# cteufel13/VisualOdometry

Measured on AMD Instinct MI355X. Metric: BA GN-iters/sec at 50 poses×20k landmarks; descriptor-match Mpairs/sec, higher is better.
Workload: dtype f64; 1 GPU; cfg3: synthetic sliding-window BA window, 50 poses x 20000 landmarks, 83108 observations (seed 3, KITTI K, first 2 poses fixed, lambda=1.0); one step = one full GN iteration; poses=50, landmarks=20000, observations=83108, parallelism=landmark-sharded x1, k1_variant=0

## Files before the change

visualodometry_amd/_lib.py:

```python

from __future__ import annotations

import ctypes as C
import os
import threading
from pathlib import Path

LIB_PATH = Path(os.environ.get("VO_LIB_PATH") or Path(__file__).resolve().parent / "lib" / "libvo_hip.so")
HEADER = Path(__file__).resolve().parents[1] / "include" / "vo_hip.h"
TEST_HEADER = HEADER.with_name("vo_hip_testing.h")

VO_OK = 0
VO_ERR_ARG = -1
VO_ERR_HIP = -2
VO_ERR_NOT_SPD = -3
VO_ERR_RCCL = -4
VO_ERR_NOMEM = -5
VO_ERR_STATE = -6
VO_ERR_NODEV = -7
VO_MATCH_DEVICE_PTRS = 1
STATUS_NAMES = {
    VO_OK: "ok", VO_ERR_ARG: "bad argument", VO_ERR_HIP: "HIP error",
    VO_ERR_NOT_SPD: "not positive definite", VO_ERR_RCCL: "RCCL error",
    VO_ERR_NOMEM: "out of device memory", VO_ERR_STATE: "bad call order",
# ... 116 lines not shown
    "vo_ba_testing_k1": (_I, [_P, _I]),
    "vo_pnp_testing_split": (_I, [_P, _I]),
    "vo_pnp_testing_group": (_I, [_P, _I]),
    "vo_pnp_testing_last_split": (_I, [_P, _PI32, _PI32]),
    "vo_ba_testing_plan_slide": (_I, [C.c_void_p, C.c_void_p, _I, _I, C.POINTER(C.c_uint64), _PI64]),
}

CHAIN_TEST_HEADER = HEADER.with_name("vo_hip_testing_chain.h")
CHAIN_SIGNATURES = {
    "vo_ba_testing_no_chain": (_I, [_P, _I]),
    "vo_ba_testing_last_run": (_I, [_P, _PI32, _PI32]),
    "vo_ba_testing_chain_poll": (_I, [_P, _I]),
    "vo_ba_testing_chain_stamps": (_I, [_P, _I, C.POINTER(C.c_uint64), _I]),
}

_lib = None
_lock = threading.Lock()


def load() -> C.CDLL:
    global _lib
    with _lock:
        if _lib is None:
            if not LIB_PATH.exists():
                raise RuntimeError(
                    f"{LIB_PATH} is missing: build it with `python -c 'import __graft_entry__ as g; g.build()'`"
                    " (hipcc --offload-arch=gfx950)"
                )
            lib = C.CDLL(str(LIB_PATH))
            tuning = bool(os.environ.get("VO_LIB_PATH"))
            for name, (res, args) in {**SIGNATURES, **CHAIN_SIGNATURES}.items():
                try:
                    fn = getattr(lib, name)
                except AttributeError:
                    if tuning:
                        continue
                    raise
                fn.restype = res
                fn.argtypes = args
            if lib.vo_abi_version() != 1:
                raise RuntimeError("libvo_hip.so ABI mismatch")
            _lib = lib
    return _lib


def check(rc: int, what: str = "") -> int:
# ... 154 lines not shown
def ba_testing_chain_poll(ctx: "Context", replicas: int = 0) -> None:
    check(ctx.lib.vo_ba_testing_chain_poll(ctx.handle, int(replicas)), "vo_ba_testing_chain_poll")


def ba_testing_chain_stamps(ctx: "Context", on: bool = True, n: int = 0):
    import numpy as np

    out = np.zeros(max(n, 1), dtype=np.uint64)
    k = ctx.lib.vo_ba_testing_chain_stamps(ctx.handle, int(bool(on)), out.ctypes.data_as(C.POINTER(C.c_uint64)),
                                           int(n))
    if k < 0:
        check(k, "vo_ba_testing_chain_stamps")
    return out[:k]


def pnp_testing_group(ctx: "Context", mode: int = 0) -> None:
    check(ctx.lib.vo_pnp_testing_group(ctx.handle, int(mode)), "vo_pnp_testing_group")


def pnp_testing_split(ctx: "Context", h1: int = 0) -> None:
    check(ctx.lib.vo_pnp_testing_split(ctx.handle, int(h1)), "vo_pnp_testing_split")


def pnp_testing_last_split(ctx: "Context") -> tuple:
    h1, tail = C.c_int32(0), C.c_int32(0)
    check(ctx.lib.vo_pnp_testing_last_split(ctx.handle, C.byref(h1), C.byref(tail)), "vo_pnp_testing_last_split")
    return h1.value, tail.value


def ptr(a, ctype):
# ... 2 lines not shown
```

visualodometry_amd/csrc/api.hip:

```cpp
#include <cstdarg>
#include <algorithm>
#include <array>
#include <cstring>
#include <vector>

#include "ba_band.h"
#include "ba_comm.h"
#include "ba_engine.h"
#include "ba_plan.h"
#include "vo_ctx.h"
#include "../../include/vo_hip_testing.h"
#include "../../include/vo_hip_testing_chain.h"

namespace vo {

namespace {
thread_local std::string g_err;
}

void set_error(const char* f, ...) {
  char buf[1024];
  va_list ap;
  va_start(ap, f);
  std::vsnprintf(buf, sizeof buf, f, ap);
  va_end(ap);
  g_err = buf;
}
// ... 1019 lines not shown
    ctx->ba_chain_poll = replicas;
  });
}

int vo_ba_testing_chain_stamps(vo_ctx* ctx, int on, uint64_t* out, int n) {
  int k = 0;
  int g = guarded([&] {
    VO_REQUIRE(ctx != nullptr, VO_ERR_ARG, "vo_ba_testing_chain_stamps: null context");
    vo::bind(ctx);
    ctx->ba_chain_stamps = on != 0;
    if (out && n > 0) k = vo::ba_chain_stamps(ctx, out, n);
  });
  return g != VO_OK ? g : k;
}

int vo_ba_testing_k1(vo_ctx* ctx, int variant) {
  return guarded([&] {
    VO_REQUIRE(ctx != nullptr, VO_ERR_ARG, "vo_ba_testing_k1: null context");
    VO_REQUIRE(variant >= -1 && variant <= vo::kWaveMaxChunks, VO_ERR_ARG, "vo_ba_testing_k1: variant %d outside -1..%d",
               variant, vo::kWaveMaxChunks);
    ctx->ba_k1_variant = variant;
  });
}

int vo_pnp_testing_group(vo_ctx* ctx, int mode) {
  return guarded([&] {
    VO_REQUIRE(ctx != nullptr, VO_ERR_ARG, "vo_pnp_testing_group: null context");
    VO_REQUIRE(mode >= -1 && mode <= 1, VO_ERR_ARG, "vo_pnp_testing_group: mode %d outside -1..1", mode);
    ctx->pnp_group = mode;
  });
// ... 46 lines not shown
```

visualodometry_amd/csrc/ba_band.h:

```cpp
#pragma once

#include <hip/hip_runtime.h>

#include <cstddef>
#include <vector>

#include "ba_kernels.h"
#include "ba_reduce.h"

namespace vo {

constexpr int kBandMaxW = 9;
constexpr int kBandMaxF = 512;
constexpr int kBandStamps = 32;
constexpr size_t kBandLdsMax = 160 * 1024 - 1024;

struct BandSplit {
  int w = 0, m = 0, nb = 0, s = 0;
};
BandSplit band_split(int F, const std::vector<int>& first);

struct BandTables {
  std::vector<int> tab;
  int merge = 0, n_merge = 0;
// ... 20 lines not shown
  double* dc;
  const double* pose_cur;
  double* pose_next;
  int* status;
  unsigned long long* stamps;
  unsigned seq;
  int nred;
  int red_drop;
  unsigned* red_count;
  const int* red_col;
  const int* col_need;
  ReduceArgs red;
  int k1_nseg = 0;
  int pub_mask = 0;
  unsigned* pub = nullptr;
  unsigned long long* k1_stamps = nullptr;
  LinArgs lin;
};
constexpr int kBandPubStride = 32;
constexpr int kBandPubReplicas = 8;
constexpr int kBandChainChunks = 6;
size_t band_chain_lds();
struct SplitXch {
  long merge, rec, z, fail, flag;
  __host__ __device__ long end() const { return flag + 3 * 16; }
};
__host__ __device__ inline SplitXch split_xch(int n_merge, int s) {
  SplitXch x;
  x.merge = 0;
  x.rec = (n_merge + 15) / 16 * 16;
  x.z = x.rec + (42L * s + 15) / 16 * 16;
  x.fail = x.z + (6L * s + 15) / 16 * 16;
  x.flag = x.fail + 16;
  return x;
}
// ... 15 lines not shown
```

visualodometry_amd/csrc/ba_band.hip:

```cpp
#include <atomic>
#include "ba_band.h"

#include <algorithm>
#include <climits>

#include "ba_lin_wave.h"
#include "ba_math.h"
#include "vo_common.h"

namespace vo {

BandSplit band_split(int F, const std::vector<int>& first) {
  BandSplit b;
  int w = 0;
  for (int i = 0; i < F; ++i) w = std::max(w, i - first[i]);
  b.w = w;
  if (F >= 2 * w + 2) {
    b.s = w;
    b.nb = (F - w) / 2;
    b.m = F - w - b.nb;
  } else {
    b.m = F;
  }
  return b;
// ... 274 lines not shown
template <int kMode, bool kLm = false, int kNext = 0>
__global__ __launch_bounds__(kBandThreads) void ba_band_kernel(BandArgs A) {
  constexpr bool kFull = kMode != 0, kSplit = kMode == 2;
  constexpr int NT = kSplit ? kBandThreads / 2 : kBandThreads;
  extern __shared__ __attribute__((aligned(16))) double dyn[];
  __shared__ int s_fail;
  __shared__ __attribute__((aligned(16))) double s_zero[40];
#if VO_BA_STAMPS
  unsigned long long st_acc[kBandStamps] = {}, st_t = __builtin_amdgcn_s_memtime();
#endif
  const int tid = threadIdx.x, wave = __builtin_amdgcn_readfirstlane(tid >> 6), lane = tid & 63;
  if constexpr (kNext != 0) {
    static_assert(kMode == 1 && !kLm, "chained: the full layout's GN launch");
    const int k1 = (int)blockIdx.x - ((int)gridDim.x - A.k1_nseg);
    if (k1 >= 0) {
      if (wave >= kBandChainChunks) return;
      LinWave* Sw = reinterpret_cast<LinWave*>(dyn);
      int* words = reinterpret_cast<int*>(Sw + kBandChainChunks);
      LinGate G;
      G.pub = A.pub + kBandPubStride * ((int)blockIdx.x & A.pub_mask);
      G.want = A.seq << 1;
      G.status = A.status;
      G.iter_tag = A.iter_tag;
      G.timeout_flag = kBandStatusTimeout;
      G.s_gate = (lin_lds_int*)(words + 1);
#if VO_BA_STAMPS
      if (A.k1_stamps) {
        G.stamps = A.k1_stamps + 2 + 4 * k1;
        if (tid == 0) G.stamps[0] = __builtin_amdgcn_s_memrealtime();
      }
#endif
      constexpr int kMode1 = kBacksub | kAccum | (kNext == 2 ? kRobust : 0);
      lin_wave_body<kMode1, false, kBandChainChunks, true>(A.lin, Sw, words, k1, G);
      return;
    }
  }
  if (A.nred > 0 && blockIdx.x > 0) {
    band_reduce_wg<kLm>(A, blockIdx.x - 1, dyn);
    return;
  }
  const int F = A.F, w = A.w, R = w + 1, CS = 36 * R + 12, CSP = (CS + 127) / 128 * 128;
  const int m = A.m, nb = A.nb, sp = A.s;
  const int ncolT = m + sp, ncolB = nb + sp;
  const int SS = kFull ? CS : CSP, RC = kFull ? max(ncolT, ncolB) : w + 4, SPAD = kFull ? 128 : 0;
// ... 726 lines not shown
      bs_go(m - 1, 0, INT_MAX);
    }
    if (role == kChain && side == 1 && nb > 0) {
      bs_init(nb + sp - 1, nb);
      bs_go(nb + sp - 1, 0, nb);
    }
  }
  BST(12);
  asm volatile("s_waitcnt lgkmcnt(0)" ::: "memory");
  __syncthreads();
  BST(13);

  const double* const recB = kFull ? ringB : A.fac + (long)ncolT * CS;
  const bool failed2 = failed || (kSplit && s_late != 0);
  auto mine = [&](int G) __attribute__((always_inline)) { return !kSplit || (G >= 0 && G >= ncolT) == sbot; };
  if (!failed2)
    for (int c = A.n_fixed + tid; c < A.n_poses; c += NT) {
      const int G = c - A.n_fixed;
      if (!mine(G)) continue;
      double* T = pose_l + 12 * c;
      const double* rec = G < ncolT ? recT + (long)G * CS : recB + (long)(F - 1 - G) * CS;
      double L[21], r[6], d[6], out[12];
#pragma unroll
      for (int ii = 0; ii < 6; ++ii)
#pragma unroll
        for (int cc = 0; cc <= ii; cc += 2) {
          const double2 v = reinterpret_cast<const double2*>(rec + 6 * ii)[cc / 2];
          L[P6(ii, cc)] = v.x;
          if (cc + 1 <= ii) L[P6(ii, cc + 1)] = v.y;
        }
      ld6g(rec + 36 * R + 6, r);
      ld6g(zs + 6 * G, d);
      bwd6(L, r, d);
      st6g(zs + 6 * G, d);
      se3_exp_apply(d, T, out);
#pragma unroll
      for (int e = 0; e < 6; ++e) reinterpret_cast<double2*>(T)[e] = make_double2(out[2 * e], out[2 * e + 1]);
    }
  asm volatile("s_waitcnt lgkmcnt(0)" ::: "memory");
  __syncthreads();
  if constexpr (kNext != 0) {
    for (int e = tid; e < 6 * A.n_poses; e += NT)
      slab_store(reinterpret_cast<double2*>(A.pose_next) + e, reinterpret_cast<const double2*>(pose_l)[e]);
    for (int e = tid; e < 3 * (A.n_poses - A.n_fixed); e += NT)
      slab_store(reinterpret_cast<double2*>(A.dc) + e,
                 failed2 ? make_double2(0.0, 0.0) : reinterpret_cast<const double2*>(zs)[e]);
    asm volatile("s_waitcnt vmcnt(0)" ::: "memory");
    __syncthreads();
    if (tid <= A.pub_mask)
      __hip_atomic_store((gu32*)(A.pub + kBandPubStride * tid), A.seq << 1 | (failed2 ? 1u : 0u), __ATOMIC_RELAXED,
                         __HIP_MEMORY_SCOPE_AGENT);
#if VO_BA_STAMPS
    if (A.k1_stamps && tid == 0) {
      A.k1_stamps[0] = __builtin_amdgcn_s_memrealtime();
      A.k1_stamps[1] = sst ? sst[0] : 0;
    }
#endif
  } else {
  for (int e = tid; e < 6 * A.n_poses; e += NT)
    if (mine(e / 6 - A.n_fixed))
      reinterpret_cast<double2*>(A.pose_next)[e] = reinterpret_cast<const double2*>(pose_l)[e];
  for (int e = tid; e < 3 * (A.n_poses - A.n_fixed); e += NT)
    if (mine(e / 3))
      reinterpret_cast<double2*>(A.dc)[e] = failed2 ? make_double2(0.0, 0.0) : reinterpret_cast<const double2*>(zs)[e];
  }
  const bool late = !reduced || (kSplit && s_late != 0);
  if (tid == 0 && (late || !kSplit || !sbot)) {
    if (late) *A.status = (prior_status ? prior_word : A.iter_tag) | kBandStatusTimeout;
    else if (failed && !prior_status) *A.status = A.iter_tag;
  }
  BST(14);
#if VO_BA_STAMPS
  if (lane == 0 && A.stamps)
// ... 57 lines not shown
```

visualodometry_amd/csrc/ba_engine.h:

```cpp
#pragma once

#include <cstdint>

#include "vo_common.h"

struct vo_ctx;

namespace vo {

uint64_t ba_setup(vo_ctx* ctx, const vo_ba_problem* p);
void ba_reserve(vo_ctx* ctx, int n_poses, int n_points, int64_t n_obs, int n_fixed);
void ba_check_session(vo_ctx* ctx, uint64_t session);
void ba_set_state(vo_ctx* ctx, const double* poses, const double* pts);
void ba_get_state(vo_ctx* ctx, double* poses, double* pts);
int ba_run(vo_ctx* ctx, int iters, double* cost, bool sync);
int ba_gn_step(vo_ctx* ctx, double* S, double* b, double* dc, double* cost);
int ba_run_lm(vo_ctx* ctx, int iters, const vo_ba_lm_options* opt, double* cost, double* lambda, double* trial,
              uint8_t* accepted, bool sync);
int ba_lm_log(vo_ctx* ctx, int n, double* cost, double* lambda, double* trial, uint8_t* accepted);
void ba_set_lm_stop(vo_ctx* ctx, const vo_ba_lm_stop* stop);
void ba_lm_stop_info(vo_ctx* ctx, int32_t* trials, int32_t* reason);
void ba_set_robust(vo_ctx* ctx, double huber_delta);
void ba_residuals(vo_ctx* ctx, double* err2, double* depth);
int ba_covariance(vo_ctx* ctx, double lambda, double* pose_cov, double* pose_dense, double* point_cov);
void ba_set_obs_weights(vo_ctx* ctx, const double* w);
void ba_get_obs_weights(vo_ctx* ctx, double* w_out);
void ba_cull(vo_ctx* ctx, const vo_ba_cull_options* opt, int32_t* n_culled, int32_t* n_active, bool sync);
int ba_stats(vo_ctx* ctx, int64_t* out, int n);
int ba_stamps(vo_ctx* ctx, uint64_t* out, int n);
int ba_chain_stamps(vo_ctx* ctx, uint64_t* out, int n);
void ba_last_run(vo_ctx* ctx, int* chained, int* launches);

}
```

visualodometry_amd/csrc/ba_engine.hip:

```cpp
#include "ba_engine.h"

#include <algorithm>
#include <atomic>
#include <cmath>
#include <cstring>
#include <string>
#include <vector>

#include "ba_band.h"
#include "ba_comm.h"
#include "ba_cov.h"
#include "ba_kernels.h"
#include "ba_plan.h"
#include "ba_weights.h"
#include "vo_ctx.h"

#ifndef VO_BA_CHAIN
#define VO_BA_CHAIN 1
#endif
#ifndef VO_BA_CHAIN_POLL
#define VO_BA_CHAIN_POLL 8
#endif
#ifndef VO_BA_FUSE
#define VO_BA_FUSE 1
// ... 752 lines not shown
  }

  void last_run(int* chained, int* launches) const {
    if (chained) *chained = last_chained_ ? 1 : 0;
    if (launches) *launches = last_launches_;
  }

  int read_chain_stamps(uint64_t* out, int n) {
    if (!stamps_on_ || !d_stamps_k1_.ptr || !last_chained_) return 0;
    const int k = std::min(n, 2 + 4 * plan_.n_segments());
    VO_HIP_CHECK(hipStreamSynchronize(ctx_->stream));
    VO_HIP_CHECK(hipMemcpy(out, d_stamps_k1_.ptr, (size_t)k * 8, hipMemcpyDeviceToHost));
    return k;
  }

  int stats(int64_t* out, int n) const {
    const BAPlan& P = plan_;
    int64_t v[12 + kSetupSections] = {P.n_chunks(), P.n_segments(), P.n_slab_slots(), (int64_t)P.slot_i.size(),
                                      P.n_prof_blocks(), P.n_te, P.algorithmic_bytes_per_iter(), band_on_ ? 1 : 0,
                                      P.reused_groups, P.reused_chunks, P.seg_obs};
    for (int i = 0; i < kSetupSections; ++i) v[11 + i] = setup_ns_[i];
    v[11 + kSetupSections] = !band_on_ ? 0 : band_lds_.split ? 3 : band_lds_.full ? 1 : 2;
    const int k = std::min(n, 12 + kSetupSections);
    for (int i = 0; i < k; ++i) out[i] = v[i];
    return k;
  }

 private:
  void require_state() const {
    VO_REQUIRE(have_problem_, VO_ERR_STATE, "BA: no problem set up");
// ... 178 lines not shown
  void upload_tables(const TablePack& pack) {
    hipStream_t st = ctx_->stream;
    h_tab_.reserve(pack.bytes);
    d_tab_.reserve(pack.bytes);
    for (const TablePack::Part& q : pack.parts)
      if (q.n) std::memcpy(h_tab_.as<char>() + q.off, q.src, q.n);
    VO_HIP_CHECK(hipMemcpyAsync(d_tab_.ptr, h_tab_.ptr, pack.bytes, hipMemcpyHostToDevice, st));
    for (const TablePack::Part& q : pack.parts) q.view->ptr = d_tab_.as<char>() + q.off;
    d_misc_.reserve(kMiscBytes);
    d_status_.ptr = d_misc_.ptr;
    d_zero_.ptr = d_misc_.as<char>() + 256;
    VO_HIP_CHECK(hipMemsetAsync(d_misc_.ptr, 0, kMiscBytes, st));
    colcnt_bytes_ = band_col_count_bytes(plan_.n_free);
    d_colcnt_.reserve(colcnt_bytes_);
    VO_HIP_CHECK(hipMemsetAsync(d_colcnt_.ptr, 0, colcnt_bytes_, st));
    d_pub_.reserve(kBandPubReplicas * kBandPubStride * sizeof(unsigned));
    VO_HIP_CHECK(hipMemsetAsync(d_pub_.ptr, 0, kBandPubReplicas * kBandPubStride * sizeof(unsigned), st));
  }

  static int segments_target(int num_cus, bool wave) {
    return wave ? (1 << 30) : VO_BA_SEGMENTS_PER_CU * std::max(1, num_cus);
  }
  static constexpr int kWaveChunksOneRound = std::min(kChunkObs >= 64 ? 6 : 8, kWaveMaxChunks),
                       kWaveChunksRounds = std::min(3, kWaveMaxChunks);
  int wave_chunks(int64_t n_obs) const {
    if (ctx_->ba_k1_variant >= 1) return std::min(ctx_->ba_k1_variant, kWaveMaxChunks);
    const int64_t one_round_obs = (int64_t)ctx_->num_cus * kWaveChunksOneRound * (kChunkObs * 7 / 8);
    return n_obs * 10 <= one_round_obs * 11 ? kWaveChunksOneRound : kWaveChunksRounds;
  }

  LinArgs lin_args() {
    const BAPlan& P = plan_;
// ... 140 lines not shown
      B.red_drop = B.nred > 0 ? ctx_->ba_drop_reducers : 0;
      B.red_count = d_colcnt_.as<unsigned>();
      B.red_col = d_red_col_.as<int>();
      B.col_need = d_col_need_.as<int>();
      B.red = reduce_args();
      if (stamps_on_) {
        d_stamps3_.reserve((8 * kBandStamps + 8 + 4 * (B.nred + 1)) * 8);
        B.stamps = d_stamps3_.as<unsigned long long>();
      }
      if (chain_next) {
        B.lin = lin_args();
        std::swap(B.lin.pose_old, B.lin.pose_new);
        B.lin.nseg = B.k1_nseg = plan_.n_segments();
        B.pub_mask = (ctx_->ba_chain_poll ? ctx_->ba_chain_poll : kChainPollReplicas) - 1;
        B.pub = d_pub_.as<unsigned>();
        if (stamps_on_) {
          d_stamps_k1_.reserve((2 + 4 * (size_t)B.k1_nseg) * 8);
          B.k1_stamps = d_stamps_k1_.as<unsigned long long>();
        }
      }
      launch_band_solve(B, band_lds_, ctx_->stream);
      return;
    }
    launch_profile_solve(A, solve_lds_, solve_lds_size_, ctx_->stream);
  }

  void enqueue_solve(int iter_tag, double* cost_slot = nullptr, bool chain_next = false) {
    const BAPlan& P = plan_;
    SolveArgs A;
    A.F = P.n_free;
    A.nprof = P.n_prof_blocks();
    A.n_poses = P.n_poses;
    A.n_fixed = P.n_fixed;
// ... 24 lines not shown
    ctx_->prof.end(ctx_->stream);
    VO_HIP_CHECK(hipGetLastError());
  }

  void iteration(double* d_cost_slot, int iter_tag, bool lin_done = false, bool chain_next = false) {
    if (!lin_done) enqueue_lin(pending_ ? (kBacksub | kAccum) : kAccum);
    enqueue_reduce();
    enqueue_solve(iter_tag, d_cost_slot, chain_next);
    cur_ ^= 1;
    pending_ = true;
  }

  bool chain_ok() const {
    const int nseg = plan_.n_segments();
    return VO_BA_CHAIN && !ctx_->ba_no_chain && band_on_ && fused() && band_lds_.full && !band_lds_.split &&
           plan_is_wave(plan_.seg_obs) && plan_.seg_chunks == kBandChainChunks && nseg > 0 &&
           (int64_t)nseg * kBandChainChunks == plan_.n_chunks() && nseg + 2 <= ctx_->num_cus && !lm_lambda_ &&
           !weighted_ &&
           !ctx_->prof.on && (!stamps_on_ || ctx_->ba_chain_stamps) && !sharded();
  }

  void finalize_cost(double* d_cost_slot) {
    enqueue_lin(pending_ ? kBacksub : 0);
    pending_ = false;
    ReduceArgs R{};
    R.nprof = 0;
    R.F = 0;
    R.nseg = std::max(1, plan_.n_segments());
    R.slab_cost = d_slab_cost_.as<double>();
    R.sys = d_cost_tmp();
// ... 32 lines not shown
  BandSplit band_{};
  bool band_on_ = false;
  bool fuse_ok_ = false;
  unsigned band_seq_ = 0;
  BandLds band_lds_;
  BandTables band_tab_;
  HostBuf h_tab_;
  DevBuf d_tab_;
  DevView d_chunk_hdr_, d_seg_hdr_, d_slab_pos_, d_cam_pos_, d_solve_tab_, d_band_tab_, d_red_meta_, d_red_out_;
  static constexpr size_t kMiscBytes = 256 + 512;
  DevBuf d_misc_;
  DevView d_status_, d_zero_;
  DevBuf d_colcnt_;
  DevBuf d_pub_;
  DevBuf d_stamps_k1_;
  static constexpr int kChainPollReplicas = VO_BA_CHAIN_POLL;
  bool last_chained_ = false;
  int last_launches_ = 0, launches_ = 0;
  size_t colcnt_bytes_ = 0;
  DevView d_red_col_, d_col_need_;
  std::vector<int32_t> red_col_, col_need_;
  std::vector<int4> red_meta_;
  std::vector<int2> red_out_;
  DevBuf d_fac_;
  std::vector<int32_t> red_dst_, red_rdst_;
  long cost_off_ = 0;
  HostBuf h_state_;
  hipEvent_t h_state_ev_ = nullptr;
  bool h_state_busy_ = false;
  DevBuf d_chunk_img_;
// ... 79 lines not shown
void ba_set_lm_stop(vo_ctx* ctx, const vo_ba_lm_stop* stop) { ba_engine(ctx)->set_lm_stop(stop); }
void ba_lm_stop_info(vo_ctx* ctx, int32_t* trials, int32_t* reason) { ba_engine(ctx)->lm_stop_info(trials, reason); }
void ba_set_robust(vo_ctx* ctx, double delta) { ba_engine(ctx)->set_robust(delta); }
void ba_residuals(vo_ctx* ctx, double* err2, double* depth) { ba_engine(ctx)->residuals(err2, depth); }
int ba_covariance(vo_ctx* ctx, double lambda, double* pose_cov, double* pose_dense, double* point_cov) {
  return ba_engine(ctx)->covariance(lambda, pose_cov, pose_dense, point_cov);
}
void ba_set_obs_weights(vo_ctx* ctx, const double* w) { ba_engine(ctx)->set_obs_weights(w); }
void ba_get_obs_weights(vo_ctx* ctx, double* w_out) { ba_engine(ctx)->get_obs_weights(w_out); }
void ba_cull(vo_ctx* ctx, const vo_ba_cull_options* opt, int32_t* n_culled, int32_t* n_active, bool sync) {
  ba_engine(ctx)->cull(opt, n_culled, n_active, sync);
}
int ba_stats(vo_ctx* ctx, int64_t* out, int n) { return ba_engine(ctx)->stats(out, n); }
int ba_stamps(vo_ctx* ctx, uint64_t* out, int n) { return ba_engine(ctx)->read_stamps(out, n); }
int ba_chain_stamps(vo_ctx* ctx, uint64_t* out, int n) { return ba_engine(ctx)->read_chain_stamps(out, n); }
void ba_last_run(vo_ctx* ctx, int* chained, int* launches) { ba_engine(ctx)->last_run(chained, launches); }

}

vo_ctx::vo_ctx() = default;

vo_ctx::~vo_ctx() {
  ba.reset();
  comm.reset();
  if (stream) (void)hipStreamDestroy(stream);
}
```

visualodometry_amd/csrc/ba_lin_wave.h:

```cpp
#pragma once

#include <hip/hip_runtime.h>

#include <cstddef>
#include <cstdint>
#include <utility>

#include "ba_kernels.h"
#include "ba_math.h"
#include "vo_common.h"

namespace vo {

namespace {

constexpr double kPivotRelEps = 1e-12;

enum { kPhLoad = 0, kPhBacksub, kPhLinObs, kPhReduce, kPhElim, kPhSchur, kPhWrite, kPhSchurU, kPhT0, kPhT1,
       kPhObs, kPhTe, kPhPts, kPhPairs, kPhSlots, kPhCams, kPhEnd };
static_assert(kPhEnd == kPhCount, "K1 stamp row (ba_kernels.h)");
template <bool kStamp>
struct Stamper {
  unsigned long long t = 0, acc[kPhCount] = {};
  bool lead = false;
// ... 316 lines not shown

__device__ __forceinline__ void slab_store(double2* p, double2 v) {
  typedef double f64x2 __attribute__((ext_vector_type(2)));
  const f64x2 d = {v.x, v.y};
  asm volatile("global_store_dwordx4 %0, %1, off sc1\n\ts_nop 0" ::"v"(p), "v"(d) : "memory");
}

typedef __attribute__((address_space(3))) int lin_lds_int;
struct LinGate {
  const unsigned* pub = nullptr;
  unsigned want = 0;
  int* status = nullptr;
  int iter_tag = 0;
  int timeout_flag = 0;
  lin_lds_int* s_gate = nullptr;
  unsigned long long* stamps = nullptr;
};
constexpr unsigned kLinGateSpins = 1u << 25;

typedef __attribute__((address_space(1))) unsigned long long lin_gu64;
typedef __attribute__((address_space(1))) unsigned lin_gu32;
__device__ __forceinline__ double ld_sc1_f64(const double* p) {
  return __longlong_as_double((long long)__hip_atomic_load((lin_gu64*)p, __ATOMIC_RELAXED, __HIP_MEMORY_SCOPE_AGENT));
}

template <int MODE, bool kStamp, int NW, bool kGated>
__device__ __forceinline__ void lin_wave_body(LinArgs A, LinWave* Sw, int* s_arrive_p, const int seg, const LinGate G,
                                              const double* sqw = nullptr) {
  int& s_arrive = *s_arrive_p;
  constexpr bool kGroup = NW > 1;
  constexpr bool kRob = (MODE & kRobust) != 0;
  constexpr bool kWt = (MODE & kWeighted) != 0;
  static_assert(!kWt || (kRob && !kGated), "weighted K1: the Huber code, never in the chained launch");
  if constexpr ((MODE & kLm) != 0) A.lambda = *A.lm_lambda;
  constexpr int kCombWaves = NW < 4 ? NW : 4;
  constexpr bool kEarly = NW > kCombWaves && (MODE & kAccum);
  constexpr int kCombS = (kSegSlots * 18 + 64 * kCombWaves - 1) / (64 * kCombWaves);
  constexpr int kCombB = (kSegCams * 3 + 64 * kCombWaves - 1) / (64 * kCombWaves);
  static_assert(kLinLanesWave == 64, "one wave");
  static_assert(!kGated || (MODE & (kBacksub | kAccum | kLm)) == (kBacksub | kAccum), "the gated K1: a GN iteration's");
  const int wv = kGroup ? __builtin_amdgcn_readfirstlane((int)threadIdx.x >> 6) : 0;
  constexpr bool kPrio = kEarly;
  if constexpr (kPrio)
    if (wv >= kCombWaves) __builtin_amdgcn_s_setprio(1);
  auto prio_drop = [&]() __attribute__((always_inline)) {
    if constexpr (kPrio)
      if (wv >= kCombWaves) __builtin_amdgcn_s_setprio(0);
  };
  LinWave& S = Sw[wv];
  const int tid = (int)threadIdx.x & 63, chk = seg * NW + wv;
  Stamper<kStamp> st;
  st.start(tid == 0, chk);
  const int* SH = A.seg_hdr + (long)kSegHdr * seg;
  const int4* SH4 = reinterpret_cast<const int4*>(SH);
  const int16_t* SH16 = reinterpret_cast<const int16_t*>(SH);
// ... 1 lines not shown
  const int4 g0 = SH4[0], g1 = SH4[1];
  const int4* CH = kGroup ? A.chunk_hdr + 4l * chk : SH4 + 8;
  const int4 h0 = CH[0], h1 = CH[1], h2 = CH[2], h3 = CH[3];
  constexpr int kImgVec = (int)(sizeof(ChunkImg) / 16);
  static_assert(kImgVec > 128 && kImgVec <= 192, "three 16-byte staging granules per lane");
  const uint4* img = reinterpret_cast<const uint4*>(A.chunk_img + chk);
  const uint4 img0 = img[tid], img1 = img[64 + tid], img2 = img[min(128 + tid, kImgVec - 1)];
  int i_acam[3], i_wcam[3];
#pragma unroll
  for (int k = 0; k < 3; ++k) {
    i_acam[k] = SH16[16 + min((tid + 64 * k) / 12, kSegAllCams - 1)];
    i_wcam[k] = SH16[32 + min((tid + 64 * k) / 6, kSegCams - 1)];
  }
  if (kEarly) {
    if (threadIdx.x == 0) s_arrive = 0;
    lds_sync_wave();
    __builtin_amdgcn_s_barrier();
    asm volatile("" ::: "memory");
  }
  if (stat) return;
  const int nslots = g0.x, slot_off = g0.y, cam0 = g0.z, ncams = g0.w, na = g1.x;
  const int nob = h0.y, nte = h0.w, p0 = h1.x, npt = h1.y;
  double* dcw = &S.zb[kZbDc];
  double* pose_o = &S.zb[kZbPoseO];
  double vx[2], vpn[3], vpo[3], vdc[3];
  const long xb = npt > 0 ? 3l * p0 : 0;
#pragma unroll
  for (int k = 0; k < 2; ++k) vx[k] = A.points[xb + min(tid + 64 * k, max(3 * npt - 1, 0))];
#pragma unroll
  for (int k = 0; k < 3; ++k) {
// ... 30 lines not shown
    if (!kGated && (MODE & kBacksub) && e < 6 * ncams) dcw[e] = vdc[k];
  }
  if (MODE & kAccum) {
    if (tid < nslots) S.spos[tid] = vsp;
    if (tid < ncams) S.cpos[tid] = vcp;
    if (kGroup) {
      S.srow[tid] = 0xFF;
      if (tid < kSegCams) S.crow[tid] = 0;
    }
  }
  if constexpr (kGated) {
#if VO_BA_STAMPS
    if (G.stamps && threadIdx.x == 0) {
      asm volatile("s_waitcnt vmcnt(0) lgkmcnt(0)" ::: "memory");
      G.stamps[1] = __builtin_amdgcn_s_memrealtime();
    }
#endif
    if (threadIdx.x == 0) {
      unsigned spins = 0, v;
      while (((v = __hip_atomic_load((lin_gu32*)G.pub, __ATOMIC_RELAXED, __HIP_MEMORY_SCOPE_AGENT)) | 1u) !=
             (G.want | 1u)) {
        __builtin_amdgcn_s_sleep(2);
        if (++spins > kLinGateSpins) break;
      }
      int verdict = (int)(v & 1u);
      if ((v | 1u) != (G.want | 1u)) {
        verdict = 1;
        const unsigned prior = __hip_atomic_load((lin_gu32*)G.status, __ATOMIC_RELAXED, __HIP_MEMORY_SCOPE_AGENT);
        __hip_atomic_fetch_or((lin_gu32*)G.status, (unsigned)G.timeout_flag | (prior ? 0u : (unsigned)G.iter_tag),
                              __ATOMIC_RELAXED, __HIP_MEMORY_SCOPE_AGENT);
      }
      *G.s_gate = verdict;
    }
    lds_sync_wave();
    __builtin_amdgcn_s_barrier();
    asm volatile("" ::: "memory");
    if (__builtin_amdgcn_readfirstlane(*(volatile lin_lds_int*)G.s_gate)) return;
#if VO_BA_STAMPS
    if (G.stamps && threadIdx.x == 0) G.stamps[2] = __builtin_amdgcn_s_memrealtime();
#endif
#pragma unroll
    for (int k = 0; k < 3; ++k) {
      const int e = tid + 64 * k;
      vpn[k] = ld_sc1_f64(A.pose_new + 12l * i_acam[k] + e % 12);
      vdc[k] = ld_sc1_f64(A.dc + 6l * i_wcam[k] + e % 6);
    }
#pragma unroll
    for (int k = 0; k < 3; ++k) {
      const int e = tid + 64 * k;
      if (e < 12 * na) (&S.pose_n[0][0])[e] = vpn[k];
      if (e < 6 * ncams) dcw[e] = vdc[k];
    }
  }
  st.count(kPhSlots, nslots);
  st.count(kPhCams, ncams);
  st.count(kPhObs, nob);
  st.count(kPhTe, nte);
  st.count(kPhPts, npt);
  st.count(kPhPairs, h2.y - h2.x);
  double cost = 0.0;
  lds_sync_wave();
  st.mark(kPhLoad);

  if (MODE & kBacksub) {
    if (tid < nob) {
      const int lc = S.img.obs_lcam[tid];
      obs_lin_w<false, true, kRob, kWt>(S, A, &pose_o[12 * S.img.acam[tid]], tid, lc >= 0 ? &dcw[6 * lc] : nullptr, cost,
// ... 4 lines not shown
      double l[6], h[3];
      if (point_block_w(S, A.lambda, tid, l, h)) {
        const double x2 = -h[2] * l[5];
        const double x1 = (-h[1] - l[4] * x2) * l[2];
        const double x0 = (-h[0] - l[1] * x1 - l[3] * x2) * l[0];
        S.X[tid][0] += x0;
        S.X[tid][1] += x1;
        S.X[tid][2] += x2;
        A.points[3l * (p0 + tid)] = S.X[tid][0];
        A.points[3l * (p0 + tid) + 1] = S.X[tid][1];
        A.points[3l * (p0 + tid) + 2] = S.X[tid][2];
      }
    }
    lds_sync_wave();
    st.mark(kPhBacksub);
  }

  if (tid < nob)
    obs_lin_w<(MODE & kAccum) != 0, false, kRob, kWt>(S, A, S.pose_n[S.img.acam[tid]], tid, nullptr, cost, sw);
  if (MODE & kAccum) {
    lds_sync_wave();
    st.mark(kPhLinObs);
    if (tid < npt) {
      double l[6], h[3];
      const bool ok = point_block_w(S, A.lambda, tid, l, h);
      S.valid[tid] = ok;
#pragma unroll
      for (int e = 0; e < 6; ++e) S.L[tid][e] = l[e];
      S.h[tid][0] = ok ? h[0] : 0.0;
      S.h[tid][1] = ok ? h[1] : 0.0;
// ... 147 lines not shown
      for (int k = 0; k < kCombB; ++k)
        if (t + 64 * kCombWaves * k < npb) slab_store(dstB[k], accB[k]);
    }
    if (t == 0) {
      double c = 0.0;
#pragma unroll
      for (int w = 0; w < NW; ++w) c += Sw[w].wcost;
      A.slab_cost[seg] = c;
    }
  }
  st.mark(kPhWrite);
  st.flush(A.stamps);
#if VO_BA_STAMPS
  if constexpr (kGated)
    if (G.stamps && threadIdx.x == 0) G.stamps[3] = __builtin_amdgcn_s_memrealtime();
#endif
}

}

}
```

visualodometry_amd/csrc/vo_ctx.h:

```cpp
#pragma once

#include <memory>
#include <vector>

#include "vo_common.h"

namespace vo {

struct MatchWorkspace {
  DevBuf des;
  DevBuf q8;
  DevBuf norms;
  DevBuf colconst;
  DevBuf partial;
  DevBuf best;
  DevBuf rev;
  DevBuf top2;
  DevBuf pairs;
  DevBuf flag;
  DevBuf tri;
  DevBuf hbf;
  DevBuf fnorm;
  DevBuf fpart;
  DevBuf bmax;
// ... 97 lines not shown
  vo::MatchWorkspace match;
  vo::MatchQueryCache match_q;
  vo::PnpWorkspace pnp;
  vo::EssWorkspace ess;
  vo::SiftWorkspace sift;
  vo::Profiler prof;
  std::unique_ptr<vo::BAEngine> ba;
  std::unique_ptr<vo::Comm> comm;
  bool ba_split_reduce = false;
  int ba_drop_reducers = 0;
  bool ba_no_split = false;
  int pnp_group = 0;
  int pnp_split = 0;
  bool ba_no_chain = false;
  int ba_chain_poll = 0;
  bool ba_chain_stamps = false;
  int ba_k1_variant = 0;
  vo_ctx();
  ~vo_ctx();
};

namespace vo {
void match_run(vo_ctx* ctx, const float* d_des0, const float* d_des1, int batch, int n0,
               int n1, int dim, double ratio, int32_t* d_best, int32_t* d_idx2,
               float* d_dist2, const MatchQueryCache* qc = nullptr, int32_t* d_rev = nullptr);
void mutual_filter(vo_ctx* ctx, int32_t* d_best, const int32_t* d_rev, int batch, int n0, int n1);
void match_pack_query(vo_ctx* ctx, const float* d_des0, int n0, int dim, MatchQueryCache& qc);
void compact_pairs(vo_ctx* ctx, const int32_t* d_best, int n0, int32_t* d_pairs,
                   int32_t* d_count);
void tri_run(vo_ctx* ctx, const double* P1, const double* P2, const double* T_cw2, const double* K,
// ... 23 lines not shown
```

Baseline: 17490 GN-iters/s.

## Split chained pose publish from dc publish with a dedicated pose-gate wave

The chained GN launch now publishes the backsubstituted pose-correction vector (dc) and the updated poses through two separate flags. Wave 1 writes dc and signals early, while wave 0 does the pose back-solve and SE3 update and signals on a second publish word. In each K1 segment block, an extra wave waits for the pose word and loads the new poses into LDS, so the backsub/accumulate stage can start on dc before the poses are ready. It also adds a pose-delay test knob, wide timestamps, and a pose-count limit on the chain path. It adds another spin-wait and more flag traffic.

```diff
diff --git a/include/vo_hip_testing_chain_pose.h b/include/vo_hip_testing_chain_pose.h
--- /dev/null
+++ b/include/vo_hip_testing_chain_pose.h
@@ -0,0 +1,17 @@
+#ifndef VO_HIP_TESTING_CHAIN_POSE_H
+#define VO_HIP_TESTING_CHAIN_POSE_H
+
+#include "vo_hip.h"
+
+#ifdef __cplusplus
+extern "C" {
+#endif
+
+int vo_ba_testing_chain_pose_delay(vo_ctx* ctx, int n);
+
+int vo_ba_testing_chain_stamps_wide(vo_ctx* ctx, uint64_t* out, int n);
+
+#ifdef __cplusplus
+}
+#endif
+#endif
diff --git a/visualodometry_amd/_lib.py b/visualodometry_amd/_lib.py
--- a/visualodometry_amd/_lib.py
+++ b/visualodometry_amd/_lib.py
@@ -154,6 +154,12 @@
     "vo_ba_testing_chain_stamps": (_I, [_P, _I, C.POINTER(C.c_uint64), _I]),
 }
 
+CHAIN_POSE_TEST_HEADER = HEADER.with_name("vo_hip_testing_chain_pose.h")
+CHAIN_POSE_SIGNATURES = {
+    "vo_ba_testing_chain_pose_delay": (_I, [_P, _I]),
+    "vo_ba_testing_chain_stamps_wide": (_I, [_P, C.POINTER(C.c_uint64), _I]),
+}
+
 _lib = None
 _lock = threading.Lock()
 
@@ -169,7 +175,7 @@
                 )
             lib = C.CDLL(str(LIB_PATH))
             tuning = bool(os.environ.get("VO_LIB_PATH"))
-            for name, (res, args) in {**SIGNATURES, **CHAIN_SIGNATURES}.items():
+            for name, (res, args) in {**SIGNATURES, **CHAIN_SIGNATURES, **CHAIN_POSE_SIGNATURES}.items():
                 try:
                     fn = getattr(lib, name)
                 except AttributeError:
@@ -354,6 +360,20 @@
     return out[:k]
 
 
+def ba_testing_chain_pose_delay(ctx: "Context", n: int = 0) -> None:
+    check(ctx.lib.vo_ba_testing_chain_pose_delay(ctx.handle, int(n)), "vo_ba_testing_chain_pose_delay")
+
+
+def ba_testing_chain_stamps_wide(ctx: "Context", n: int = 0):
+    import numpy as np
+
+    out = np.zeros(max(n, 1), dtype=np.uint64)
+    k = ctx.lib.vo_ba_testing_chain_stamps_wide(ctx.handle, out.ctypes.data_as(C.POINTER(C.c_uint64)), int(n))
+    if k < 0:
+        check(k, "vo_ba_testing_chain_stamps_wide")
+    return out[:k]
+
+
 def pnp_testing_group(ctx: "Context", mode: int = 0) -> None:
     check(ctx.lib.vo_pnp_testing_group(ctx.handle, int(mode)), "vo_pnp_testing_group")
 
diff --git a/visualodometry_amd/csrc/api.hip b/visualodometry_amd/csrc/api.hip
--- a/visualodometry_amd/csrc/api.hip
+++ b/visualodometry_amd/csrc/api.hip
@@ -11,6 +11,7 @@
 #include "vo_ctx.h"
 #include "../../include/vo_hip_testing.h"
 #include "../../include/vo_hip_testing_chain.h"
+#include "../../include/vo_hip_testing_chain_pose.h"
 
 namespace vo {
 
@@ -1060,6 +1061,24 @@
   return g != VO_OK ? g : k;
 }
 
+int vo_ba_testing_chain_pose_delay(vo_ctx* ctx, int n) {
+  return guarded([&] {
+    VO_REQUIRE(ctx != nullptr, VO_ERR_ARG, "vo_ba_testing_chain_pose_delay: null context");
+    VO_REQUIRE(n >= 0 && n <= 64, VO_ERR_ARG, "vo_ba_testing_chain_pose_delay: %d sleeps outside 0..64", n);
+    ctx->ba_chain_pose_delay = n;
+  });
+}
+
+int vo_ba_testing_chain_stamps_wide(vo_ctx* ctx, uint64_t* out, int n) {
+  int k = 0;
+  int g = guarded([&] {
+    VO_REQUIRE(ctx != nullptr, VO_ERR_ARG, "vo_ba_testing_chain_stamps_wide: null context");
+    vo::bind(ctx);
+    if (out && n > 0) k = vo::ba_chain_stamps_wide(ctx, out, n);
+  });
+  return g != VO_OK ? g : k;
+}
+
 int vo_ba_testing_k1(vo_ctx* ctx, int variant) {
   return guarded([&] {
     VO_REQUIRE(ctx != nullptr, VO_ERR_ARG, "vo_ba_testing_k1: null context");
diff --git a/visualodometry_amd/csrc/ba_band.h b/visualodometry_amd/csrc/ba_band.h
--- a/visualodometry_amd/csrc/ba_band.h
+++ b/visualodometry_amd/csrc/ba_band.h
@@ -58,11 +58,15 @@
   int k1_nseg = 0;
   int pub_mask = 0;
   unsigned* pub = nullptr;
+  int pose_delay = 0;
   unsigned long long* k1_stamps = nullptr;
+  unsigned long long* k1_wide = nullptr;
   LinArgs lin;
 };
 constexpr int kBandPubStride = 32;
 constexpr int kBandPubReplicas = 8;
+constexpr int kBandPubB = kBandPubReplicas * kBandPubStride;
+constexpr int kBandChainPoses = 64;
 constexpr int kBandChainChunks = 6;
 size_t band_chain_lds();
 struct SplitXch {
diff --git a/visualodometry_amd/csrc/ba_band.hip b/visualodometry_amd/csrc/ba_band.hip
--- a/visualodometry_amd/csrc/ba_band.hip
+++ b/visualodometry_amd/csrc/ba_band.hip
@@ -312,20 +312,30 @@
     static_assert(kMode == 1 && !kLm, "chained: the full layout's GN launch");
     const int k1 = (int)blockIdx.x - ((int)gridDim.x - A.k1_nseg);
     if (k1 >= 0) {
-      if (wave >= kBandChainChunks) return;
+      if (wave > kBandChainChunks) return;
       LinWave* Sw = reinterpret_cast<LinWave*>(dyn);
       int* words = reinterpret_cast<int*>(Sw + kBandChainChunks);
       LinGate G;
       G.pub = A.pub + kBandPubStride * ((int)blockIdx.x & A.pub_mask);
+      G.pub_b = G.pub + kBandPubB;
       G.want = A.seq << 1;
       G.status = A.status;
       G.iter_tag = A.iter_tag;
       G.timeout_flag = kBandStatusTimeout;
       G.s_gate = (lin_lds_int*)(words + 1);
+      G.s_pose = (lin_lds_int*)(words + 2);
+      if (wave == kBandChainChunks) {
+        lin_pose_wave<kBandChainChunks>(A.lin, Sw, k1, G);
+        return;
+      }
 #if VO_BA_STAMPS
       if (A.k1_stamps) {
         G.stamps = A.k1_stamps + 2 + 4 * k1;
         if (tid == 0) G.stamps[0] = __builtin_amdgcn_s_memrealtime();
+      }
+      if (A.k1_wide) {
+        G.wide = A.k1_wide + 4 + 8 * k1;
+        if (tid == 0) G.wide[0] = __builtin_amdgcn_s_memrealtime();
       }
 #endif
       constexpr int kMode1 = kBacksub | kAccum | (kNext == 2 ? kRobust : 0);
@@ -1082,6 +1092,74 @@
   const double* const recB = kFull ? ringB : A.fac + (long)ncolT * CS;
   const bool failed2 = failed || (kSplit && s_late != 0);
   auto mine = [&](int G) __attribute__((always_inline)) { return !kSplit || (G >= 0 && G >= ncolT) == sbot; };
+  if constexpr (kNext != 0) {
+    const int c = lane, G = c - A.n_fixed;
+    const bool row = wave == 0 && c < A.n_poses, upd = row && G >= 0 && !failed2;
+    double d[6], out[12];
+    const double* T = pose_l + 12 * (row ? c : 0);
+    if (wave == 0) {
+#pragma unroll
+      for (int e = 0; e < 6; ++e) {
+        const double2 v = reinterpret_cast<const double2*>(T)[e];
+        out[2 * e] = v.x;
+        out[2 * e + 1] = v.y;
+      }
+      if (upd) {
+        const double* rec = G < ncolT ? recT + (long)G * CS : recB + (long)(F - 1 - G) * CS;
+        double L[21], r[6];
+#pragma unroll
+        for (int ii = 0; ii < 6; ++ii)
+#pragma unroll
+          for (int cc = 0; cc <= ii; cc += 2) {
+            const double2 v = reinterpret_cast<const double2*>(rec + 6 * ii)[cc / 2];
+            L[P6(ii, cc)] = v.x;
+            if (cc + 1 <= ii) L[P6(ii, cc + 1)] = v.y;
+          }
+        ld6g(rec + 36 * R + 6, r);
+        ld6g(zs + 6 * G, d);
+        bwd6(L, r, d);
+        st6g(zs + 6 * G, d);
+      }
+    }
+    band_barrier();
+    const unsigned word = A.seq << 1 | (failed2 ? 1u : 0u);
+    if (wave == 0) {
+      if (upd) se3_exp_apply(d, T, out);
+      if (row) {
+#pragma unroll
+        for (int e = 0; e < 6; ++e)
+          slab_store(reinterpret_cast<double2*>(A.pose_next) + 6 * c + e, make_double2(out[2 * e], out[2 * e + 1]));
+      }
+      asm volatile("s_waitcnt vmcnt(0)" ::: "memory");
+      for (int i = 0; i < A.pose_delay; ++i) __builtin_amdgcn_s_sleep(127);
+      if (lane <= A.pub_mask)
+        __hip_atomic_store((gu32*)(A.pub + kBandPubB + kBandPubStride * lane), word, __ATOMIC_RELAXED,
+                           __HIP_MEMORY_SCOPE_AGENT);
+#if VO_BA_STAMPS
+      if (A.k1_stamps && tid == 0) {
+        A.k1_stamps[0] = __builtin_amdgcn_s_memrealtime();
+        A.k1_stamps[1] = sst ? sst[0] : 0;
+      }
+      if (A.k1_wide && tid == 0) {
+        A.k1_wide[1] = __builtin_amdgcn_s_memrealtime();
+        A.k1_wide[2] = sst ? sst[0] : 0;
+        unsigned xcc, hw;
+        asm volatile("s_getreg_b32 %0, hwreg(HW_REG_XCC_ID)\n\ts_getreg_b32 %1, hwreg(HW_REG_HW_ID)" : "=s"(xcc), "=s"(hw));
+        A.k1_wide[3] = (unsigned long long)hw << 32 | xcc;
+      }
+#endif
+    } else if (wave == 1) {
+      for (int e = lane; e < 3 * (A.n_poses - A.n_fixed); e += 64)
+        slab_store(reinterpret_cast<double2*>(A.dc) + e,
+                   failed2 ? make_double2(0.0, 0.0) : reinterpret_cast<const double2*>(zs)[e]);
+      asm volatile("s_waitcnt vmcnt(0)" ::: "memory");
+      if (lane <= A.pub_mask)
+        __hip_atomic_store((gu32*)(A.pub + kBandPubStride * lane), word, __ATOMIC_RELAXED, __HIP_MEMORY_SCOPE_AGENT);
+#if VO_BA_STAMPS
+      if (A.k1_wide && lane == 0) A.k1_wide[0] = __builtin_amdgcn_s_memrealtime();
+#endif
+    }
+  } else {
   if (!failed2)
     for (int c = A.n_fixed + tid; c < A.n_poses; c += NT) {
       const int G = c - A.n_fixed;
@@ -1107,24 +1185,6 @@
     }
   asm volatile("s_waitcnt lgkmcnt(0)" ::: "memory");
   __syncthreads();
-  if constexpr (kNext != 0) {
-    for (int e = tid; e < 6 * A.n_poses; e += NT)
-      slab_store(reinterpret_cast<double2*>(A.pose_next) + e, reinterpret_cast<const double2*>(pose_l)[e]);
-    for (int e = tid; e < 3 * (A.n_poses - A.n_fixed); e += NT)
-      slab_store(reinterpret_cast<double2*>(A.dc) + e,
-                 failed2 ? make_double2(0.0, 0.0) : reinterpret_cast<const double2*>(zs)[e]);
-    asm volatile("s_waitcnt vmcnt(0)" ::: "memory");
-    __syncthreads();
-    if (tid <= A.pub_mask)
-      __hip_atomic_store((gu32*)(A.pub + kBandPubStride * tid), A.seq << 1 | (failed2 ? 1u : 0u), __ATOMIC_RELAXED,
-                         __HIP_MEMORY_SCOPE_AGENT);
-#if VO_BA_STAMPS
-    if (A.k1_stamps && tid == 0) {
-      A.k1_stamps[0] = __builtin_amdgcn_s_memrealtime();
-      A.k1_stamps[1] = sst ? sst[0] : 0;
-    }
-#endif
-  } else {
   for (int e = tid; e < 6 * A.n_poses; e += NT)
     if (mine(e / 6 - A.n_fixed))
       reinterpret_cast<double2*>(A.pose_next)[e] = reinterpret_cast<const double2*>(pose_l)[e];
diff --git a/visualodometry_amd/csrc/ba_engine.h b/visualodometry_amd/csrc/ba_engine.h
--- a/visualodometry_amd/csrc/ba_engine.h
+++ b/visualodometry_amd/csrc/ba_engine.h
@@ -29,6 +29,7 @@
 int ba_stats(vo_ctx* ctx, int64_t* out, int n);
 int ba_stamps(vo_ctx* ctx, uint64_t* out, int n);
 int ba_chain_stamps(vo_ctx* ctx, uint64_t* out, int n);
+int ba_chain_stamps_wide(vo_ctx* ctx, uint64_t* out, int n);
 void ba_last_run(vo_ctx* ctx, int* chained, int* launches);
 
 }
diff --git a/visualodometry_amd/csrc/ba_engine.hip b/visualodometry_amd/csrc/ba_engine.hip
--- a/visualodometry_amd/csrc/ba_engine.hip
+++ b/visualodometry_amd/csrc/ba_engine.hip
@@ -790,6 +790,14 @@
     return k;
   }
 
+  int read_chain_stamps_wide(uint64_t* out, int n) {
+    if (!stamps_on_ || !d_stamps_wide_.ptr || !last_chained_) return 0;
+    const int k = std::min(n, 4 + 8 * plan_.n_segments());
+    VO_HIP_CHECK(hipStreamSynchronize(ctx_->stream));
+    VO_HIP_CHECK(hipMemcpy(out, d_stamps_wide_.ptr, (size_t)k * 8, hipMemcpyDeviceToHost));
+    return k;
+  }
+
   int stats(int64_t* out, int n) const {
     const BAPlan& P = plan_;
     int64_t v[12 + kSetupSections] = {P.n_chunks(), P.n_segments(), P.n_slab_slots(), (int64_t)P.slot_i.size(),
@@ -998,8 +1006,8 @@
     colcnt_bytes_ = band_col_count_bytes(plan_.n_free);
     d_colcnt_.reserve(colcnt_bytes_);
     VO_HIP_CHECK(hipMemsetAsync(d_colcnt_.ptr, 0, colcnt_bytes_, st));
-    d_pub_.reserve(kBandPubReplicas * kBandPubStride * sizeof(unsigned));
-    VO_HIP_CHECK(hipMemsetAsync(d_pub_.ptr, 0, kBandPubReplicas * kBandPubStride * sizeof(unsigned), st));
+    d_pub_.reserve(2 * kBandPubB * sizeof(unsigned));
+    VO_HIP_CHECK(hipMemsetAsync(d_pub_.ptr, 0, 2 * kBandPubB * sizeof(unsigned), st));
   }
 
   static int segments_target(int num_cus, bool wave) {
@@ -1170,9 +1178,12 @@
         B.lin.nseg = B.k1_nseg = plan_.n_segments();
         B.pub_mask = (ctx_->ba_chain_poll ? ctx_->ba_chain_poll : kChainPollReplicas) - 1;
         B.pub = d_pub_.as<unsigned>();
+        B.pose_delay = ctx_->ba_chain_pose_delay;
         if (stamps_on_) {
           d_stamps_k1_.reserve((2 + 4 * (size_t)B.k1_nseg) * 8);
           B.k1_stamps = d_stamps_k1_.as<unsigned long long>();
+          d_stamps_wide_.reserve((4 + 8 * (size_t)B.k1_nseg) * 8);
+          B.k1_wide = d_stamps_wide_.as<unsigned long long>();
         }
       }
       launch_band_solve(B, band_lds_, ctx_->stream);
@@ -1227,6 +1238,7 @@
   bool chain_ok() const {
     const int nseg = plan_.n_segments();
     return VO_BA_CHAIN && !ctx_->ba_no_chain && band_on_ && fused() && band_lds_.full && !band_lds_.split &&
+           plan_.n_poses <= kBandChainPoses &&
            plan_is_wave(plan_.seg_obs) && plan_.seg_chunks == kBandChainChunks && nseg > 0 &&
            (int64_t)nseg * kBandChainChunks == plan_.n_chunks() && nseg + 2 <= ctx_->num_cus && !lm_lambda_ &&
            !weighted_ &&
@@ -1289,6 +1301,7 @@
   DevBuf d_colcnt_;
   DevBuf d_pub_;
   DevBuf d_stamps_k1_;
+  DevBuf d_stamps_wide_;
   static constexpr int kChainPollReplicas = VO_BA_CHAIN_POLL;
   bool last_chained_ = false;
   int last_launches_ = 0, launches_ = 0;
@@ -1398,6 +1411,7 @@
 int ba_stats(vo_ctx* ctx, int64_t* out, int n) { return ba_engine(ctx)->stats(out, n); }
 int ba_stamps(vo_ctx* ctx, uint64_t* out, int n) { return ba_engine(ctx)->read_stamps(out, n); }
 int ba_chain_stamps(vo_ctx* ctx, uint64_t* out, int n) { return ba_engine(ctx)->read_chain_stamps(out, n); }
+int ba_chain_stamps_wide(vo_ctx* ctx, uint64_t* out, int n) { return ba_engine(ctx)->read_chain_stamps_wide(out, n); }
 void ba_last_run(vo_ctx* ctx, int* chained, int* launches) { ba_engine(ctx)->last_run(chained, launches); }
 
 }
diff --git a/visualodometry_amd/csrc/ba_lin_wave.h b/visualodometry_amd/csrc/ba_lin_wave.h
--- a/visualodometry_amd/csrc/ba_lin_wave.h
+++ b/visualodometry_amd/csrc/ba_lin_wave.h
@@ -354,7 +354,10 @@
   int iter_tag = 0;
   int timeout_flag = 0;
   lin_lds_int* s_gate = nullptr;
+  const unsigned* pub_b = nullptr;
+  lin_lds_int* s_pose = nullptr;
   unsigned long long* stamps = nullptr;
+  unsigned long long* wide = nullptr;
 };
 constexpr unsigned kLinGateSpins = 1u << 25;
 
@@ -362,6 +365,51 @@
 typedef __attribute__((address_space(1))) unsigned lin_gu32;
 __device__ __forceinline__ double ld_sc1_f64(const double* p) {
   return __longlong_as_double((long long)__hip_atomic_load((lin_gu64*)p, __ATOMIC_RELAXED, __HIP_MEMORY_SCOPE_AGENT));
+}
+
+template <int NW>
+__device__ __forceinline__ void lin_pose_wave(const LinArgs& A, LinWave* Sw, const int seg, const LinGate& G) {
+  const int tid = (int)threadIdx.x & 63;
+  const int* SH = A.seg_hdr + (long)kSegHdr * seg;
+  const int16_t* SH16 = reinterpret_cast<const int16_t*>(SH);
+  const int na = reinterpret_cast<const int4*>(SH)[1].x;
+  int i_acam[3];
+#pragma unroll
+  for (int k = 0; k < 3; ++k) i_acam[k] = SH16[16 + min((tid + 64 * k) / 12, kSegAllCams - 1)];
+  lds_sync_wave();
+  __builtin_amdgcn_s_barrier();
+  lds_sync_wave();
+  __builtin_amdgcn_s_barrier();
+  asm volatile("" ::: "memory");
+  if (__builtin_amdgcn_readfirstlane(*(volatile lin_lds_int*)G.s_gate)) return;
+  unsigned spins = 0, v;
+  while (((v = __builtin_amdgcn_readfirstlane(
+               __hip_atomic_load((lin_gu32*)G.pub_b, __ATOMIC_RELAXED, __HIP_MEMORY_SCOPE_AGENT))) |
+          1u) != (G.want | 1u)) {
+    __builtin_amdgcn_s_sleep(2);
+    if (++spins > kLinGateSpins) break;
+  }
+  int word = 2;
+  if (v == G.want) {
+    double vpn[3];
+#pragma unroll
+    for (int k = 0; k < 3; ++k) vpn[k] = ld_sc1_f64(A.pose_new + 12l * i_acam[k] + (tid + 64 * k) % 12);
+#pragma unroll
+    for (int k = 0; k < 3; ++k) {
+      const int e = tid + 64 * k;
+      if (e < 12 * na)
+#pragma unroll
+        for (int w = 0; w < NW; ++w) (&Sw[w].pose_n[0][0])[e] = vpn[k];
+    }
+    lds_sync_wave();
+    word = 1;
+  } else if ((v | 1u) != (G.want | 1u) && tid == 0) {
+    const unsigned prior = __hip_atomic_load((lin_gu32*)G.status, __ATOMIC_RELAXED, __HIP_MEMORY_SCOPE_AGENT);
+    __hip_atomic_fetch_or((lin_gu32*)G.status, (unsigned)G.timeout_flag | (prior ? 0u : (unsigned)G.iter_tag),
+                          __ATOMIC_RELAXED, __HIP_MEMORY_SCOPE_AGENT);
+  }
+  if (tid == 0) *(volatile lin_lds_int*)G.s_pose = word;
+  lds_sync_wave();
 }
 
 template <int MODE, bool kStamp, int NW, bool kGated>
@@ -379,6 +427,7 @@
   constexpr int kCombB = (kSegCams * 3 + 64 * kCombWaves - 1) / (64 * kCombWaves);
   static_assert(kLinLanesWave == 64, "one wave");
   static_assert(!kGated || (MODE & (kBacksub | kAccum | kLm)) == (kBacksub | kAccum), "the gated K1: a GN iteration's");
+  static_assert(!kGated || kEarly, "the gated K1's pose wave joins the arrival word's barrier and the gate's");
   const int wv = kGroup ? __builtin_amdgcn_readfirstlane((int)threadIdx.x >> 6) : 0;
   constexpr bool kPrio = kEarly;
   if constexpr (kPrio)
@@ -410,6 +459,8 @@
   }
   if (kEarly) {
     if (threadIdx.x == 0) s_arrive = 0;
+    if constexpr (kGated)
+      if (threadIdx.x == 0) *(volatile lin_lds_int*)G.s_pose = 0;
     lds_sync_wave();
     __builtin_amdgcn_s_barrier();
     asm volatile("" ::: "memory");
@@ -470,6 +521,7 @@
     if (G.stamps && threadIdx.x == 0) {
       asm volatile("s_waitcnt vmcnt(0) lgkmcnt(0)" ::: "memory");
       G.stamps[1] = __builtin_amdgcn_s_memrealtime();
+      if (G.wide) G.wide[1] = G.stamps[1];
     }
 #endif
     if (threadIdx.x == 0) {
@@ -494,19 +546,13 @@
     if (__builtin_amdgcn_readfirstlane(*(volatile lin_lds_int*)G.s_gate)) return;
 #if VO_BA_STAMPS
     if (G.stamps && threadIdx.x == 0) G.stamps[2] = __builtin_amdgcn_s_memrealtime();
+    if (G.wide && threadIdx.x == 0) G.wide[2] = __builtin_amdgcn_s_memrealtime();
 #endif
 #pragma unroll
-    for (int k = 0; k < 3; ++k) {
-      const int e = tid + 64 * k;
-      vpn[k] = ld_sc1_f64(A.pose_new + 12l * i_acam[k] + e % 12);
-      vdc[k] = ld_sc1_f64(A.dc + 6l * i_wcam[k] + e % 6);
-    }
-#pragma unroll
-    for (int k = 0; k < 3; ++k) {
-      const int e = tid + 64 * k;
-      if (e < 12 * na) (&S.pose_n[0][0])[e] = vpn[k];
-      if (e < 6 * ncams) dcw[e] = vdc[k];
-    }
+    for (int k = 0; k < 3; ++k) vdc[k] = ld_sc1_f64(A.dc + 6l * i_wcam[k] + (tid + 64 * k) % 6);
+#pragma unroll
+    for (int k = 0; k < 3; ++k)
+      if (tid + 64 * k < 6 * ncams) dcw[tid + 64 * k] = vdc[k];
   }
   st.count(kPhSlots, nslots);
   st.count(kPhCams, ncams);
@@ -541,6 +587,18 @@
     }
     lds_sync_wave();
     st.mark(kPhBacksub);
+    if constexpr (kGated) {
+#if VO_BA_STAMPS
+      if (G.wide && threadIdx.x == 0) G.wide[3] = __builtin_amdgcn_s_memrealtime();
+#endif
+      int pw;
+      while ((pw = __builtin_amdgcn_readfirstlane(*(volatile lin_lds_int*)G.s_pose)) == 0) __builtin_amdgcn_s_sleep(1);
+      asm volatile("" ::: "memory");
+      if (pw != 1) return;
+#if VO_BA_STAMPS
+      if (G.wide && threadIdx.x == 0) G.wide[4] = __builtin_amdgcn_s_memrealtime();
+#endif
+    }
   }
 
   if (tid < nob)
@@ -718,6 +776,14 @@
 #if VO_BA_STAMPS
   if constexpr (kGated)
     if (G.stamps && threadIdx.x == 0) G.stamps[3] = __builtin_amdgcn_s_memrealtime();
+  if constexpr (kGated)
+    if (G.wide && threadIdx.x == 0) {
+      unsigned xcc, hw;
+      asm volatile("s_getreg_b32 %0, hwreg(HW_REG_XCC_ID)\n\ts_getreg_b32 %1, hwreg(HW_REG_HW_ID)" : "=s"(xcc), "=s"(hw));
+      G.wide[5] = __builtin_amdgcn_s_memrealtime();
+      G.wide[6] = xcc;
+      G.wide[7] = hw;
+    }
 #endif
 }
 
diff --git a/visualodometry_amd/csrc/vo_ctx.h b/visualodometry_amd/csrc/vo_ctx.h
--- a/visualodometry_amd/csrc/vo_ctx.h
+++ b/visualodometry_amd/csrc/vo_ctx.h
@@ -135,6 +135,7 @@
   int pnp_split = 0;
   bool ba_no_chain = false;
   int ba_chain_poll = 0;
+  int ba_chain_pose_delay = 0;
   bool ba_chain_stamps = false;
   int ba_k1_variant = 0;
   vo_ctx();
```

Result: no change. 17590 GN-iters/s, median of 6 (+0.6%).
